# togatoga/kanpyo

Measured on AMD Instinct MI355X. Metric: sentences/sec, higher is better.
Workload: dtype i32; 1 GPU; BASELINE configs[1] (cfg 2): 100k synthetic ~40-char sentences, batch 4096, IPADIC-shaped 392k-record dictionary; batch=4096, batches_in_flight=8, streams=3, long_streams=0, GPU_MAX_HW_QUEUES=4, residency=inputs resident in HBM, dense tokens left in HBM

## Files before the change

### kanpyo_amd/csrc/kgpu_chain.cpp

```cpp
#include "kgpu_chain.h"

#include <algorithm>
#include <cstdlib>

namespace kgpu {

LaunchPlan make_launch_plan(int cus, const Occupancy &occ) {
    LaunchPlan t{};
    t.general_workgroups = cus * 2;
    const char *e = getenv("KGPU_POOL");
    t.pool_limit_auto = e == nullptr;
    for (const char *q = e ? e : "40:4:32"; *q && t.n_pools < 2;) {
        int kib = atoi(q), w = 8, mp = 64;
        const char *c = q;
        while (*c && *c != ',' && *c != ':') ++c;
        if (*c == ':' && atoi(c + 1) > 0) {
            w = atoi(c + 1);
            ++c;
            while (*c && *c != ',' && *c != ':') ++c;
            if (*c == ':' && atoi(c + 1) > 0) mp = atoi(c + 1);
        }
        w = std::min(w, 16);
        mp = std::min(mp, 64);
        const int per_cu = kib >= 8 && kib <= 160 ? occ.pool((uint32_t)kib * 1024, (uint32_t)w) : 0;
        if (per_cu > 0) {
            t.pool_bytes[t.n_pools] = (uint32_t)kib * 1024; t.pool_waves[t.n_pools] = (uint32_t)w;
            t.pool_max_pages[t.n_pools] = (uint32_t)mp;
            t.pool_workgroups[t.n_pools] = cus * per_cu;
            ++t.n_pools;
        }
        while (*q && *q != ',') ++q;
        if (*q == ',') ++q;
    }
    t.alt_pool_bytes = 20 * 1024; t.alt_pool_waves = 2;
    const int alt_per_cu = (t.pool_limit_auto && t.n_pools) ? occ.pool(t.alt_pool_bytes, t.alt_pool_waves) : 0;
    t.alt_pool_workgroups = alt_per_cu > 0 ? cus * alt_per_cu : 0;
    const char *w = getenv("KGPU_WINDOW");
    int kib = w ? atoi(w) : 10;
    if (kib < 8 || kib > 160) kib = 0;
    t.window_lds_bytes = (uint32_t)kib * 1024;
    const int per_cu = kib ? occ.window(t.window_lds_bytes) : 0;
    t.window_workgroups = cus * per_cu;
    if (per_cu <= 0) t.window_lds_bytes = 0;
    t.window_team_workgroups = t.window_lds_bytes ? cus * std::max(0, occ.window_team(t.window_lds_bytes)) : 0;
    const char *tm = getenv("KGPU_WINDOW_TEAM");
    t.window_team_mode = tm ? atoi(tm) : -1;
    const char *wf = getenv("KGPU_WINDOW_FIRST");
    t.window_first_bytes = (uint32_t)std::max(0, wf ? atoi(wf) : 1024);
    return t;
}

int Chain::pools() const {
    int k = 0;
    while (k < n && steps[k].kernel == Kernel::Pool) ++k;
    return k;
}
const Step *Chain::find(Kernel k) const {
    for (int i = 0; i < n; ++i) if (steps[i].kernel == k) return &steps[i];
    return nullptr;
}

bool starts_with_window(const LaunchPlan &plan, const Batch &b) {
    const uint64_t lim = plan.window_first_bytes;
    return lim && b.n && plan.n_pools && plan.window_lds_bytes && !b.dump && b.stop_after == 0 && !b.no_window && b.bytes >= lim * b.n;
}

static Step window_step(const LaunchPlan &plan, uint64_t n, int in, int out, int grid_est) {
    uint64_t wg = plan.window_workgroups;
    if (in < 0 && n < wg) wg = n;
    if (in >= 0 && grid_est > 0 && (uint64_t)grid_est < wg) wg = (uint64_t)grid_est;
    const uint64_t expected = in >= 0 ? (grid_est > 64 ? ((uint64_t)grid_est - 64) * 4 / 5 : 0) : n;
    return Step{Kernel::Window, in, out, (int)(wg ? wg : 1), plan.window_lds_bytes, 1, 0, expected > wg};
}
static Step general_step(const LaunchPlan &plan, uint64_t n, int in) {
    uint64_t wg = plan.general_workgroups;
    if (in < 0 && n < wg) wg = n;
    return Step{Kernel::General, in, -1, (int)(wg ? wg : 1), 0, 0, 0, false};
}

Chain build_chain(const LaunchPlan &plan, const Batch &b, Steering &st, ContextSteering &cs) {
    Chain ch;
    if (!b.n) return ch;
    const int pools = starts_with_window(plan, b) ? 0 : st.big_pool_batches.load(std::memory_order_relaxed) > 0 ? plan.n_pools : std::min(plan.n_pools, 1);
    const bool window = plan.window_lds_bytes && !b.no_window && !b.dump && b.stop_after == 0 &&
                        (pools == 0 || st.window_batches.load(std::memory_order_relaxed) > 0);
    const bool general = (pools == 0 && !window) || b.stop_after != 0 || b.dump || b.no_window || st.tail_batches.load(std::memory_order_relaxed) > 0;
    bool team = false;
    if (pools == 0 && window && plan.window_team_workgroups > 0 && plan.window_team_mode != 0) {
// ... 79 lines not shown
```

### kanpyo_amd/csrc/kgpu_chain.h

```cpp
#pragma once
#include <atomic>
#include <cstdint>

#include "kgpu_internal.h"

namespace kgpu {

struct LaunchPlan {
    int n_pools;
    uint32_t pool_bytes[2];
    uint32_t pool_waves[2];
    uint32_t pool_max_pages[2];
    bool pool_limit_auto;
    uint32_t alt_pool_bytes, alt_pool_waves;
    int alt_pool_workgroups;
    int pool_workgroups[2];
    int general_workgroups;
    uint32_t window_lds_bytes;
    int window_workgroups;
    int window_team_workgroups;
    int window_team_mode;
    uint32_t window_first_bytes;
};

struct Occupancy {
    int (*pool)(uint32_t pool_bytes, uint32_t waves);
    int (*window)(uint32_t lds_bytes);
    int (*window_team)(uint32_t lds_bytes);
};
LaunchPlan make_launch_plan(int compute_units, const Occupancy &occ);

enum class Kernel : uint8_t { Pool, WindowTeam, Window, General };
struct Step {
    Kernel kernel;
    int in;
    int out;
    int grid;
    uint32_t lds_bytes;
    uint32_t waves;
    uint32_t max_pages;
    bool claim;
};

struct Chain {
    Step steps[4];
    int n = 0;
    bool event_behind_first = false;
    bool small_scan = false;
    bool aux_one_launch = false;
    int pools() const;
    const Step *find(Kernel k) const;
    int last_list() const { return n ? steps[n - 1].out : -1; }
};

constexpr uint64_t AUX_ONE_LAUNCH_MAX = 4096;

struct Batch {
    uint64_t n, bytes;
    uint32_t est_q8;
    uint32_t stop_after;
    bool dump;
    bool no_window;
    bool share_known;
};

struct Steering {
    std::atomic<uint32_t> est_q8{64 * 256};
    std::atomic<int> big_pool_batches{0};
    std::atomic<int> window_batches{64};
    std::atomic<int> tail_batches{0};
    std::atomic<int> long_sentences_in_flight{0};
    std::atomic<int> long_peak{0};
};
struct ContextSteering {
    uint32_t win_share_q8 = 0;
    bool long_share = false;
    int counted_long = 0;
};

bool starts_with_window(const LaunchPlan &plan, const Batch &b);
Chain build_chain(const LaunchPlan &plan, const Batch &b, Steering &st, ContextSteering &cs);
Chain tail_chain(const LaunchPlan &plan, const Chain &ran);
void chain_feedback(const LaunchPlan &plan, const Chain &ran, const Chain *tail, const Control &h, uint64_t n, uint32_t est_q8, Steering &st,
                    ContextSteering &cs);

}
```

### kanpyo_amd/csrc/kgpu_ctx.cpp

```cpp
#include <algorithm>
#include <cstdlib>
#include <cstring>
#include <mutex>
#include <vector>

#include "kgpu_runtime.h"


extern "C" int kgpu_ctx_create(kgpu_dict *d, void *hip_stream, kgpu_ctx **out) {
    if (!d || !out) { set_error("kgpu_ctx_create: null argument"); return KGPU_ERR_INVALID_ARG; }
    *out = nullptr;
    HIPCHECK(hipSetDevice(d->device));
    kgpu_ctx *c = new kgpu_ctx();
    c->dict = d;
    d->refs.fetch_add(1, std::memory_order_relaxed);
    if (hip_stream) { c->stream = (hipStream_t)hip_stream; c->own_stream = true; }
    else {
        std::lock_guard<std::mutex> g(d->pool_mu);
        const unsigned n_streams = planned_streams();
        if (d->streams.size() < n_streams) {
            hipStream_t st = nullptr;
            hipError_t e = hipStreamCreateWithFlags(&st, hipStreamNonBlocking);
            if (e != hipSuccess) { set_error("hipStreamCreate: %s", hipGetErrorString(e)); kgpu_ctx_destroy(c); return KGPU_ERR_HIP; }
            d->streams.push_back(st);
            c->stream = st;
        } else {
            c->stream = d->streams[d->next_stream++ % d->streams.size()];
        }
        c->short_stream = c->stream;
    }
    if (hipMalloc((void **)&c->d_ctl, sizeof(Control)) != hipSuccess ||
        hipHostMalloc((void **)&c->h_ctl, sizeof(Control), hipHostMallocMapped) != hipSuccess ||
        hipHostGetDevicePointer((void **)&c->h_ctl_dev, c->h_ctl, 0) != hipSuccess) {
        set_error("kgpu_ctx_create: control block allocation failed");
        kgpu_ctx_destroy(c);
        return KGPU_ERR_HIP;
    }
    if (hipEventCreateWithFlags(&c->done_ev, hipEventDisableTiming) != hipSuccess || hipEventCreateWithFlags(&c->switch_ev, hipEventDisableTiming) != hipSuccess) {
        set_error("kgpu_ctx_create: hipEventCreate failed");
        kgpu_ctx_destroy(c);
        return KGPU_ERR_HIP;
    }
    hipDeviceProp_t p;
    const int cus = hipGetDeviceProperties(&p, d->device) == hipSuccess ? p.multiProcessorCount : 256;
    c->plan = make_launch_plan(cus, Occupancy{pool_workgroups_per_cu, window_workgroups_per_cu, window_team_workgroups_per_cu});
    c->aux_mode = test_hooks().aux_launch;
    *out = c;
    return KGPU_OK;
}

static void ctx_retire(kgpu_ctx *c) {
    c->pending = false;
    if (c->steer.counted_long) { c->dict->steer.long_sentences_in_flight.fetch_sub(c->steer.counted_long, std::memory_order_relaxed); c->steer.counted_long = 0; }
}

extern "C" void kgpu_ctx_destroy(kgpu_ctx *c) {
    if (!c) return;
    (void)hipSetDevice(c->dict->device);
    if (c->pending && c->done_ev) (void)hipEventSynchronize(c->done_ev);
    ctx_retire(c);
    if (c->done_ev) (void)hipEventDestroy(c->done_ev);
    c->lines_report.release(); c->split_report.release();
    c->lines_len.release(); c->lines_text.release(); c->lines_off.release(); c->lines_status.release();
    c->split_agg.release(); c->split_raw.release(); c->split_text.release(); c->split_off.release();
    c->gv_desc.release(); c->gv_len.release(); c->gv_text.release(); c->norm_text.release();
    if (c->switch_ev) (void)hipEventDestroy(c->switch_ev);
    for (auto e : c->ev_pool) (void)hipEventDestroy(e);
    c->arena.release(); c->ovf.release(); c->stat_slots.release(); c->stage.release(); c->tok_count.release();
    c->in_utf8.release(); c->in_off.release(); c->out_tok.release(); c->out_off.release(); c->out_status.release();
    c->pin_in.release(); c->pin_out.release(); c->in_block.release();
    if (c->d_ctl) (void)hipFree(c->d_ctl);
    if (c->h_ctl) (void)hipHostFree(c->h_ctl);
    if (c->sm_host) (void)hipHostFree(c->sm_host);
    kgpu_dict *d = c->dict;
    delete c;
    dict_release(d);
}

static int next_event(kgpu_ctx *c, hipEvent_t *ev) {
    if (c->ev_used == c->ev_pool.size()) {
        hipEvent_t e;
        HIPCHECK(hipEventCreate(&e));
        c->ev_pool.push_back(e);
    }
    *ev = c->ev_pool[c->ev_used++];
    return KGPU_OK;
}

static int ctx_pick_stream(kgpu_ctx *c, const Batch &b) {
    if (c->own_stream) { c->h2d_queued = false; return KGPU_OK; }
    hipStream_t want = c->short_stream;
    if ((starts_with_window(c->plan, b) || c->steer.long_share) && planned_long_streams()) {
        if (!c->long_stream) {
            kgpu_dict *d = c->dict;
            std::lock_guard<std::mutex> g(d->pool_mu);
            if (d->long_streams.size() < planned_long_streams()) {
                hipStream_t st = nullptr;
                if (hipStreamCreateWithFlags(&st, hipStreamNonBlocking) == hipSuccess) d->long_streams.push_back(st);
                else (void)hipGetLastError();
            }
            if (!d->long_streams.empty()) c->long_stream = d->long_streams[d->next_long++ % d->long_streams.size()];
        }
        if (c->long_stream) want = c->long_stream;
    }
    if (want != c->stream) {
        if (c->h2d_queued) {
            HIPCHECK(hipEventRecord(c->switch_ev, c->stream));
            HIPCHECK(hipStreamWaitEvent(want, c->switch_ev, 0));
        }
        c->stream = want;
    }
    c->h2d_queued = false;
    return KGPU_OK;
}

static int run_chain(kgpu_ctx *c, const BatchArgs &a, const hipEvent_t *ev, const char *what) {
    const Chain &ch = c->chain;
    if (ev && !ch.event_behind_first) HIPCHECK(hipEventRecord(ev[0], c->stream));
    for (int k = 0; k < ch.n; ++k) {
        hipError_t e = (hipError_t)launch_step(c->dict->view, a, ch.steps[k], c->stop_after, c->stream);
        if (e == hipSuccess && ev && k == 0 && ch.event_behind_first) e = hipEventRecord(ev[0], c->stream);
        if (e != hipSuccess) { set_error("%s launch: %s", what, hipGetErrorString(e)); return KGPU_ERR_HIP; }
    }
    if (ev) HIPCHECK(hipEventRecord(ev[1], c->stream));
    c->h_ctl->pack_overflow = 0;
    hipError_t e = (hipError_t)launch_scan_compact(a, c->h_ctl_dev, c->stream, ch.small_scan, ch.aux_one_launch, c->aux_mode, &c->aux_form);
    if (e != hipSuccess) { set_error("scan/compact launch: %s", hipGetErrorString(e)); return KGPU_ERR_HIP; }
    if (ev) HIPCHECK(hipEventRecord(ev[2], c->stream));
    HIPCHECK(hipEventRecord(c->done_ev, c->stream));
    c->ctl_dirty = false;
    c->pending = true;
    return KGPU_OK;
}

static int enqueue(kgpu_ctx *c, const BatchArgs &a, const Batch &b) {
    if (c->ctl_dirty) HIPCHECK(hipMemsetAsync(c->d_ctl, 0, sizeof(Control), c->stream));
    c->ctl_dirty = true;
    hipEvent_t ev[4] = {};
    int rc;
    const bool timed = c->profiling && (c->launch_seq++ % c->event_every) == 0;
    if (timed) {
        for (hipEvent_t &e : ev) if ((rc = next_event(c, &e))) return rc;
        HIPCHECK(hipEventRecord(ev[0], c->stream));
    }
    c->chain = build_chain(c->plan, b, c->dict->steer, c->steer);
    c->last = a;
    return run_chain(c, a, timed ? ev + 1 : nullptr, "k_tokenize");
}

int kgpu::tokenize_device_impl(kgpu_ctx *c, const uint8_t *d_utf8, const uint64_t *d_offsets, uint64_t n, uint64_t total_bytes,
                                kgpu_token *d_tokens, kgpu_token8 *d_tokens8, uint32_t *d_first, uint8_t *status8, uint64_t *toff8, uint64_t token_capacity,
                                uint64_t *d_tok_offsets, uint8_t *d_status, const char *who) {
    if (!c || !d_offsets || !d_tok_offsets || (n && !d_status) || (total_bytes && !d_utf8) ||
        (token_capacity && !d_tokens && !d_tokens8) || (d_tokens8 && n && !d_first)) {
        set_error("%s: null argument", who);
        return KGPU_ERR_INVALID_ARG;
    }
    if (n >= (1ull << 32) - 1) { set_error("%s: more than 2^32-2 sentences in one batch; split it", who); return KGPU_ERR_INVALID_ARG; }
    if (total_bytes >= (1ull << 32)) { set_error("%s: batch larger than 4 GiB; split it", who); return KGPU_ERR_INVALID_ARG; }
    HIPCHECK(hipSetDevice(c->dict->device));
    int rc;
    if (c->pending && (rc = kgpu_ctx_sync(c, nullptr)) != KGPU_OK && rc != KGPU_ERR_CAPACITY) return rc;
    const Batch b{n, total_bytes, c->dict->steer.est_q8.load(std::memory_order_relaxed), c->stop_after, false, false, c->rt.batches > 0};
    if ((rc = ctx_pick_stream(c, b))) return rc;
    if ((rc = c->arena.ensure(ARENA_INITIAL)) || (rc = c->stage.ensure((size_t)token_bound(total_bytes, n) * sizeof(kgpu_token) + 64)) ||
        (rc = c->tok_count.ensure((size_t)(n + 1) * 4)) ||
        (rc = c->ovf.ensure((size_t)(n + 1) * 4 * 4)))
        return rc;
    BatchArgs a{};
    a.utf8 = d_utf8; a.offsets = d_offsets; a.n = n; a.ctl = c->d_ctl;
    a.arena = (uint8_t *)c->arena.p; a.arena_bytes = c->arena.bytes;
    a.stage = (kgpu_token *)c->stage.p;
    a.tok_count = (uint32_t *)c->tok_count.p;
    a.status = d_status; a.out = d_tokens; a.out_cap = token_capacity; a.tok_offsets = d_tok_offsets;
    a.out8 = d_tokens8; a.first8 = d_first; a.status8 = status8; a.toff8 = toff8;
    a.count_work = c->count_work ? (c->count_no_t ? 3u : 1u) : 0u;
#ifdef KGPU_STEP_TIMING
    const bool want_stats = true;
#else
    const bool want_stats = c->count_work;
#endif
    if (want_stats) {
        if (!c->stat_slots.p) {
            if ((rc = c->stat_slots.ensure((size_t)STAT_SLOTS * STAT_WORDS * 8))) return rc;
            HIPCHECK(hipMemsetAsync(c->stat_slots.p, 0, (size_t)STAT_SLOTS * STAT_WORDS * 8, c->stream));
        }
        a.stat_slots = (unsigned long long *)c->stat_slots.p;
    }
    a.est_q8 = b.est_q8;
    for (int k = 0; k < 4; ++k) a.ovf[k] = (uint32_t *)c->ovf.p + (size_t)k * (n + 1);
    c->batch = b;
    return enqueue(c, a, b);
}

static int enqueue_tail(kgpu_ctx *c, int li) {
    HIPCHECK(hipMemcpyAsync(&c->d_ctl->ovf_count[li], &c->tail_saved.ovf_count[li], sizeof(unsigned), hipMemcpyHostToDevice, c->stream));
    c->ctl_dirty = true;
    return run_chain(c, c->last, nullptr, "tail");
}

extern "C" int kgpu_tokenize_device(kgpu_ctx *c, const uint8_t *d_utf8, const uint64_t *d_offsets, uint64_t n,
                                    uint64_t total_bytes, kgpu_token *d_tokens, uint64_t token_capacity,
                                    uint64_t *d_tok_offsets, uint8_t *d_status) {
    return tokenize_device_impl(c, d_utf8, d_offsets, n, total_bytes, d_tokens, nullptr, nullptr, nullptr, nullptr, token_capacity, d_tok_offsets, d_status,
                                "kgpu_tokenize_device");
}

extern "C" int kgpu_tokenize_device_compact(kgpu_ctx *c, const uint8_t *d_utf8, const uint64_t *d_offsets, uint64_t n,
                                            uint64_t total_bytes, kgpu_token8 *d_tokens8, uint64_t token_capacity,
                                            uint32_t *d_first, uint64_t *d_tok_offsets, uint8_t *d_status) {
    if (token_capacity && !d_tokens8) { set_error("kgpu_tokenize_device_compact: null argument"); return KGPU_ERR_INVALID_ARG; }
    return tokenize_device_impl(c, d_utf8, d_offsets, n, total_bytes, nullptr, d_tokens8, d_first, nullptr, nullptr, token_capacity, d_tok_offsets, d_status,
                                "kgpu_tokenize_device_compact");
}

extern "C" void kgpu_expand_tokens(const kgpu_token8 *in, const uint64_t *tok_offsets, const uint32_t *first, uint64_t n, kgpu_token *out) {
    const bool stream = n && expand_stream_wanted(tok_offsets[n] - tok_offsets[0]);
    expand_tokens(in, tok_offsets, first, n, out, stream);
    if (stream) expand_fence();
}

extern "C" int kgpu_ctx_sync(kgpu_ctx *c, uint64_t *n_tokens) {
    if (!c) { set_error("kgpu_ctx_sync: null ctx"); return KGPU_ERR_INVALID_ARG; }
    HIPCHECK(hipSetDevice(c->dict->device));
    for (;;) {
        if (!c->pending) { if (n_tokens) *n_tokens = 0; return KGPU_OK; }
        HIPCHECK(hipEventSynchronize(c->done_ev));
        if (c->h_ctl->window_fail && !c->h_ctl->arena_overflow) {
            c->rt.window_reruns++;
            if (c->last.stat_slots) HIPCHECK(hipMemsetAsync(c->last.stat_slots, 0, (size_t)STAT_SLOTS * STAT_WORDS * 8, c->stream));
            c->tail_pass = false;
            Batch b = c->batch;
            b.no_window = true;
            int rc = enqueue(c, c->last, b);
            if (rc) { ctx_retire(c); return rc; }
            continue;
        }
        const int li = c->chain.last_list();
        if (li >= 0 && !c->h_ctl->arena_overflow && c->h_ctl->ovf_count[li] > 0) {
            c->rt.tail_reruns++;
            c->tail_saved = *c->h_ctl;
            c->tail_pass = true;
            c->first_pass = c->chain;
            c->chain = tail_chain(c->plan, c->first_pass);
            int rc = enqueue_tail(c, li);
            if (rc) { ctx_retire(c); c->tail_pass = false; return rc; }
            continue;
        }
        if (c->h_ctl->arena_overflow) {
            size_t want = c->arena.bytes * 2;
            if (want > ARENA_MAX) { set_error("scratch arena exceeded %zu bytes", ARENA_MAX); ctx_retire(c); return KGPU_ERR_INTERNAL; }
            int rc = c->arena.ensure(want);
            if (rc) { ctx_retire(c); return rc; }
            BatchArgs a = c->last;
            a.arena = (uint8_t *)c->arena.p; a.arena_bytes = c->arena.bytes;
            c->rt.arena_regrows++;
            c->tail_pass = false;
            if (a.stat_slots) HIPCHECK(hipMemsetAsync(a.stat_slots, 0, (size_t)STAT_SLOTS * STAT_WORDS * 8, c->stream));
            if ((rc = enqueue(c, a, c->batch))) { ctx_retire(c); return rc; }
            continue;
        }
        break;
    }
    ctx_retire(c);
    const Chain &first = c->tail_pass ? c->first_pass : c->chain;
    const Chain *tail = c->tail_pass ? &c->chain : nullptr;
    if (c->tail_pass) {
        c->tail_pass = false;
        Control &h = *c->h_ctl;
        const Control &sv = c->tail_saved;
        for (int k = 0; k < 4; ++k) { if (k <= first.last_list()) h.ovf_count[k] = sv.ovf_count[k]; h.late_count[k] += sv.late_count[k]; }
        for (int k = 0; k < 7; ++k) h.work[k] += sv.work[k];
        for (int k = 0; k < 10; ++k) h.phase[k] += sv.phase[k];
        h.pack_overflow |= sv.pack_overflow;
    }
    c->rt.batches++; c->rt.sentences += c->last.n;
    for (int k = 0; k < 4; ++k) { c->rt.deferred[k] += c->h_ctl->ovf_count[k]; c->rt.redone[k] += c->h_ctl->late_count[k]; }
    if (first.find(Kernel::Window) || (tail && tail->find(Kernel::Window))) c->rt.long_launches++;
    chain_feedback(c->plan, first, tail, *c->h_ctl, c->last.n, c->last.est_q8, c->dict->steer, c->steer);
    if (c->profiling) {
        for (size_t i = 0; i + 4 <= c->ev_used; i += 4) {
            float t0f = 0, t01 = 0, t12 = 0;
            if (hipEventElapsedTime(&t0f, c->ev_pool[i], c->ev_pool[i + 1]) == hipSuccess &&
                hipEventElapsedTime(&t01, c->ev_pool[i], c->ev_pool[i + 2]) == hipSuccess &&
                hipEventElapsedTime(&t12, c->ev_pool[i + 2], c->ev_pool[i + 3]) == hipSuccess) {
                c->prof.launches++; c->rt.first_ms += t0f; c->prof.tokenize_ms += t01; c->prof.aux_ms += t12;
            }
        }
        c->ev_used = 0;
    }
    if (c->last.count_work) {
        const unsigned long long *w = c->h_ctl->work;
        c->work.sentences += w[0]; c->work.B += w[1]; c->work.C += w[2]; c->work.T += w[3];
        c->work.N += w[4]; c->work.E += w[5]; c->work.K += w[6];
        for (int k = 0; k < 10; ++k) c->phase[k] += c->h_ctl->phase[k];
    }
    if (c->last.stat_slots) {
        const size_t words = (size_t)STAT_SLOTS * STAT_WORDS;
        c->stat_host.resize(words);
        HIPCHECK(hipMemcpyAsync(c->stat_host.data(), c->last.stat_slots, words * 8, hipMemcpyDeviceToHost, c->stream));
        HIPCHECK(hipMemsetAsync(c->last.stat_slots, 0, words * 8, c->stream));
        HIPCHECK(hipStreamSynchronize(c->stream));
        unsigned long long sum[STAT_WORDS] = {0};
        for (size_t i = 0; i < words; ++i) sum[i % STAT_WORDS] += c->stat_host[i];
        c->work.sentences += sum[0]; c->work.B += sum[1]; c->work.C += sum[2]; c->work.T += sum[3];
        c->work.N += sum[4]; c->work.E += sum[5]; c->work.K += sum[6];
        for (int k = 0; k < 10; ++k) c->phase[k] += sum[16 + k];
    }
    uint64_t need = c->h_ctl->n_tokens;
    if (c->last.out8 && c->h_ctl->pack_overflow) {
        if (n_tokens) *n_tokens = 0;
        set_error("a token does not fit the 8-byte record (more than 4095 chars or 262143 bytes): use the 24-byte form for this batch");
        return KGPU_ERR_CAPACITY;
    }
    if (n_tokens) *n_tokens = need;
    if (c->h_ctl->n_tokens > c->last.out_cap) {
        set_error("token buffer too small: need %llu, capacity %llu", (unsigned long long)need, (unsigned long long)c->last.out_cap);
        return KGPU_ERR_CAPACITY;
    }
    return KGPU_OK;
}

extern "C" int kgpu_debug_aux_form(kgpu_ctx *c) { return c ? c->aux_form : -1; }

extern "C" int kgpu_ctx_set_profiling(kgpu_ctx *c, int mode) {
    if (!c) { set_error("kgpu_ctx_set_profiling: null ctx"); return KGPU_ERR_INVALID_ARG; }
    c->profiling = (mode & KGPU_PROFILE_EVENTS) != 0;
    c->event_every = (mode & KGPU_PROFILE_SAMPLED) ? 4u : 1u;
    c->launch_seq = 0;
    c->count_work = (mode & KGPU_PROFILE_WORK) != 0;
    c->count_no_t = (mode & KGPU_PROFILE_NO_T) != 0;
    return KGPU_OK;
}

extern "C" int kgpu_ctx_set_ablation(kgpu_ctx *c, int stop_after_stage) {
    if (!c || stop_after_stage < 0 || stop_after_stage > 7) { set_error("kgpu_ctx_set_ablation: bad argument"); return KGPU_ERR_INVALID_ARG; }
    c->stop_after = (uint32_t)stop_after_stage;
    return KGPU_OK;
}

extern "C" int kgpu_ctx_get_phase_cycles(kgpu_ctx *c, uint64_t out[10], int reset) {
    if (!c || !out) { set_error("kgpu_ctx_get_phase_cycles: null argument"); return KGPU_ERR_INVALID_ARG; }
    for (int k = 0; k < 10; ++k) { out[k] = c->phase[k]; if (reset) c->phase[k] = 0; }
    return KGPU_OK;
}

extern "C" int kgpu_ctx_get_work(kgpu_ctx *c, kgpu_work *out, int reset) {
    if (!c || !out) { set_error("kgpu_ctx_get_work: null argument"); return KGPU_ERR_INVALID_ARG; }
    *out = c->work;
    if (reset) c->work = kgpu_work{};
    return KGPU_OK;
}

extern "C" int kgpu_ctx_get_profile(kgpu_ctx *c, kgpu_profile *out, int reset) {
    if (!c || !out) { set_error("kgpu_ctx_get_profile: null argument"); return KGPU_ERR_INVALID_ARG; }
    *out = c->prof;
    if (reset) c->prof = kgpu_profile{};
    return KGPU_OK;
}

extern "C" int kgpu_ctx_get_plan(kgpu_ctx *c, kgpu_plan_info *out, size_t out_size) {
    if (!c || !out || out_size < 4) { set_error("kgpu_ctx_get_plan: bad argument"); return KGPU_ERR_INVALID_ARG; }
    HIPCHECK(hipSetDevice(c->dict->device));
    kgpu_plan_info p{};
    hipDeviceProp_t prop;
    p.compute_units = hipGetDeviceProperties(&prop, c->dict->device) == hipSuccess ? (uint32_t)prop.multiProcessorCount : 0u;
    if (c->plan.n_pools) {
        p.pool_lds_bytes = c->plan.pool_bytes[0]; p.pool_wavefronts = c->plan.pool_waves[0]; p.pool_max_pages = c->plan.pool_max_pages[0];
        p.pool_workgroups_per_cu = (uint32_t)pool_workgroups_per_cu(c->plan.pool_bytes[0], c->plan.pool_waves[0]);
    }
    p.window_lds_bytes = c->plan.window_lds_bytes; p.window_workgroups = (uint32_t)c->plan.window_workgroups;
    p.window_workgroups_per_cu = c->plan.window_lds_bytes ? (uint32_t)window_workgroups_per_cu(c->plan.window_lds_bytes) : 0u;
    p.streams = planned_streams();
    p.long_streams = c->own_stream ? 0u : planned_long_streams();
    p.window_first_bytes = (c->plan.n_pools && c->plan.window_lds_bytes) ? c->plan.window_first_bytes : 0u;
    std::memcpy(out, &p, std::min(out_size, sizeof p));
    return KGPU_OK;
}

extern "C" int kgpu_ctx_get_routing(kgpu_ctx *c, kgpu_routing *out, size_t out_size, int reset) {
    if (!c || !out || out_size < 8) { set_error("kgpu_ctx_get_routing: bad argument"); return KGPU_ERR_INVALID_ARG; }
    std::memcpy(out, &c->rt, std::min(out_size, sizeof(kgpu_routing)));
    if (reset) c->rt = kgpu_routing{};
    return KGPU_OK;
}

int HostReport::arm() {
    if (pending) { pending = false; HIPCHECK(hipEventSynchronize(ev)); }
    if (int rc = ctl.ensure(16, true)) return rc;
    if (!ev) HIPCHECK(hipEventCreateWithFlags(&ev, hipEventDisableTiming));
    unsigned long long *h = (unsigned long long *)ctl.h;
    h[0] = 0; h[1] = 0;
    return KGPU_OK;
}
int HostReport::record(hipStream_t stream, uint64_t cap_) {
    HIPCHECK(hipEventRecord(ev, stream));
    pending = true;
    cap = cap_;
    return KGPU_OK;
}
int HostReport::wait(uint64_t words[2]) {
    pending = false;
    HIPCHECK(hipEventSynchronize(ev));
    const unsigned long long *h = (const unsigned long long *)ctl.h;
    words[0] = h[0]; words[1] = h[1];
    return KGPU_OK;
// ... 1 lines not shown
void HostReport::release() {
    if (pending && ev) (void)hipEventSynchronize(ev);
    if (ev) (void)hipEventDestroy(ev);
    ev = nullptr; pending = false;
    ctl.release();
}

int kgpu::require_features(kgpu_dict *d, const char *who) {
    std::lock_guard<std::mutex> g(d->feat_mu);
    if (!d->feat) { set_error("%s: the dictionary has no feature tables: call kgpu_dict_set_features first", who); return KGPU_ERR_INVALID_ARG; }
    return KGPU_OK;
}
int kgpu::begin_records_call(kgpu_ctx *c, const char *who) {
    if (c->pending) { set_error("%s: the context's tokenize batch is not synced (kgpu_ctx_sync) yet", who); return KGPU_ERR_INVALID_ARG; }
    HIPCHECK(hipSetDevice(c->dict->device));
    int rc;
    if (c->lines_report.pending && (rc = kgpu_ctx_sync_lines(c, nullptr)) != KGPU_OK && rc != KGPU_ERR_CAPACITY) return rc;
    return KGPU_OK;
}
int kgpu::records_batch(kgpu_ctx *c, const DeviceRecords &r, size_t scratch_bytes, uint64_t *d_unit_offsets, RecordsBatch &b) {
    int rc;
    if ((rc = c->lines_report.arm()) || (rc = c->lines_len.ensure(scratch_bytes))) return rc;
    const kgpu_dict_info &di = c->dict->info;
    b = RecordsBatch{r.d_utf8, r.d_offsets, r.n, r.d_tokens, r.d_tok_offsets, (uint32_t)di.n_morphs, (uint32_t)(di.n_morphs + di.n_unk_morphs),
                     (uint64_t *)c->lines_len.p, d_unit_offsets, r.status_in, r.status_out, c->lines_report.dev()};
    return KGPU_OK;
}
int kgpu::records_launched(kgpu_ctx *c, int launch_error, const char *who, const char *what, uint64_t capacity) {
    if (launch_error != (int)hipSuccess) { set_error("%s: %s launch: %s", who, what, hipGetErrorString((hipError_t)launch_error)); return KGPU_ERR_HIP; }
    return c->lines_report.record(c->stream, capacity);
}
int kgpu::enqueue_lines(kgpu_ctx *c, const DeviceRecords &r, uint8_t *d_text, uint64_t text_capacity, uint64_t *d_text_offsets, const char *who) {
    kgpu_dict *d = c->dict;
    LinesArgs a{};
    int rc;
    if ((rc = require_features(d, who)) || (rc = records_batch(c, r, (size_t)r.n * 8 + 8, d_text_offsets, a.b))) return rc;
    a.feat = d->feat; a.feat_off = d->feat_off;
    a.text = d_text; a.text_cap = text_capacity;
    return records_launched(c, launch_format_lines(a, c->stream), who, "render", text_capacity);
}

extern "C" int kgpu_format_lines_device(kgpu_ctx *c, const uint8_t *d_utf8, const uint64_t *d_offsets, uint64_t n,
                                        const kgpu_token *d_tokens, const uint64_t *d_tok_offsets,
                                        uint8_t *d_text, uint64_t text_capacity, uint64_t *d_text_offsets) {
    const char *who = "kgpu_format_lines_device";
    if (!c || !d_offsets || !d_tok_offsets || !d_text_offsets || (n && (!d_utf8 || !d_tokens)) || (text_capacity && !d_text)) {
        set_error("%s: null argument", who);
        return KGPU_ERR_INVALID_ARG;
    }
    if (int rc = begin_records_call(c, who)) return rc;
    return enqueue_lines(c, DeviceRecords{d_utf8, d_offsets, n, d_tokens, d_tok_offsets, nullptr, nullptr}, d_text, text_capacity, d_text_offsets, who);
}

extern "C" int kgpu_ctx_sync_lines(kgpu_ctx *c, uint64_t *n_bytes) {
    if (!c) { set_error("kgpu_ctx_sync_lines: null ctx"); return KGPU_ERR_INVALID_ARG; }
    if (!c->lines_report.pending) { if (n_bytes) *n_bytes = 0; return KGPU_OK; }
    HIPCHECK(hipSetDevice(c->dict->device));
    uint64_t h[2];
    if (int rc = c->lines_report.wait(h)) return rc;
    const uint64_t need = h[0];
    if (n_bytes) *n_bytes = need;
    if (h[1]) {
        set_error("kgpu_ctx_sync_lines: a token record names a class, morph id or surface outside the dictionary or its sentence");
        return KGPU_ERR_INVALID_ARG;
    }
    if (need > c->lines_report.cap) {
        set_error("text buffer too small: need %llu, capacity %llu", (unsigned long long)need, (unsigned long long)c->lines_report.cap);
        return KGPU_ERR_CAPACITY;
    }
    return KGPU_OK;
}

int kgpu::pool_get(kgpu_dict *d, kgpu_ctx **out) {
    kgpu_ctx *c = nullptr;
    {
        std::lock_guard<std::mutex> g(d->pool_mu);
        if (!d->pool.empty()) { c = d->pool.back(); d->pool.pop_back(); }
    }
    if (!c) { int rc = kgpu_ctx_create(d, nullptr, &c); if (rc) return rc; }
    *out = c;
    return KGPU_OK;
}
void kgpu::pool_put(kgpu_dict *d, kgpu_ctx *c) {
    std::lock_guard<std::mutex> g(d->pool_mu);
    d->pool.push_back(c);
}

int kgpu::ctx_h2d(kgpu_ctx *c, void *dst, const void *src, size_t bytes, const char *what) {
    const hipError_t e = hipMemcpyAsync(dst, src, bytes, hipMemcpyHostToDevice, c->stream);
    if (e != hipSuccess) { set_error("%s: %s", what, hipGetErrorString(e)); return KGPU_ERR_HIP; }
    c->h2d_queued = true;
    return KGPU_OK;
}

extern "C" int kgpu_lattice_dump(kgpu_dict *d, const uint8_t *utf8, uint64_t len, kgpu_lattice *out) {
    if (!d || !out || (len && !utf8)) { set_error("kgpu_lattice_dump: null argument"); return KGPU_ERR_INVALID_ARG; }
    if (len >= (1ull << 31)) { set_error("kgpu_lattice_dump: sentence too long"); return KGPU_ERR_INVALID_ARG; }
    *out = kgpu_lattice{};
    HIPCHECK(hipSetDevice(d->device));
    PooledCtx lease(d);
    kgpu_ctx *c = lease.c;
    int rc = lease.rc;
    if (rc) return rc;
    const uint64_t offs[2] = {0, len};
    Control hc{};
    if ((c->pending && (rc = kgpu_ctx_sync(c, nullptr)) != KGPU_OK && rc != KGPU_ERR_CAPACITY) ||
        (rc = c->arena.ensure(ARENA_INITIAL)) || (rc = c->stage.ensure((size_t)(len + 2) * sizeof(kgpu_token) + 64)) ||
        (rc = c->tok_count.ensure(8)) || (rc = c->in_utf8.ensure((size_t)len + 16)) || (rc = c->in_off.ensure(16)) ||
        (rc = c->out_status.ensure(16))) return rc;
    auto fail = [&](hipError_t e, const char *what) { set_error("kgpu_lattice_dump: %s: %s", what, hipGetErrorString(e)); c->ctl_dirty = true; return KGPU_ERR_HIP; };
    hipError_t e;
    if (len && (e = hipMemcpyAsync(c->in_utf8.p, utf8, (size_t)len, hipMemcpyHostToDevice, c->stream)) != hipSuccess) return fail(e, "H2D");
    if ((e = hipMemcpyAsync(c->in_off.p, offs, 16, hipMemcpyHostToDevice, c->stream)) != hipSuccess) return fail(e, "H2D");
    for (;;) {
        BatchArgs a{};
        a.utf8 = (const uint8_t *)c->in_utf8.p; a.offsets = (const uint64_t *)c->in_off.p; a.n = 1; a.ctl = c->d_ctl;
        a.arena = (uint8_t *)c->arena.p; a.arena_bytes = c->arena.bytes;
        a.stage = (kgpu_token *)c->stage.p; a.tok_count = (uint32_t *)c->tok_count.p; a.status = (uint8_t *)c->out_status.p;
        a.dump_lattice = 1;
        c->ctl_dirty = true;
        if ((e = hipMemsetAsync(c->d_ctl, 0, sizeof(Control), c->stream)) != hipSuccess) return fail(e, "memset");
        if ((e = (hipError_t)launch_general_only(d->view, a, c->stream)) != hipSuccess) return fail(e, "launch");
        if ((e = hipMemcpyAsync(&hc, c->d_ctl, sizeof(Control), hipMemcpyDeviceToHost, c->stream)) != hipSuccess) return fail(e, "D2H");
        if ((e = hipStreamSynchronize(c->stream)) != hipSuccess) return fail(e, "sync");
        if (!hc.arena_overflow) break;
        size_t want = c->arena.bytes * 2;
        if (want > ARENA_MAX) { set_error("scratch arena exceeded %zu bytes", ARENA_MAX); return KGPU_ERR_INTERNAL; }
        if ((rc = c->arena.ensure(want))) return rc;
    }
    if (!hc.dump[5]) { set_error("kgpu_lattice_dump: the sentence is not valid UTF-8"); return KGPU_ERR_INVALID_ARG; }
    const uint64_t B = hc.dump[2], C = hc.dump[3], N = hc.dump[4], na = B + 4;
    std::vector<uint32_t> cbyte(C + 1), boff(C + 2), pre(N);
    std::vector<uint32_t> nodeA(4 * N), bucket(4 * N), nodeB(2 * N);
    const uint8_t *sa = (const uint8_t *)c->arena.p + hc.dump[0], *sn = (const uint8_t *)c->arena.p + hc.dump[1];
    if ((e = hipMemcpy(cbyte.data(), sa, (C + 1) * 4, hipMemcpyDeviceToHost)) != hipSuccess ||
        (e = hipMemcpy(boff.data(), sa + 3 * na * 4, (C + 2) * 4, hipMemcpyDeviceToHost)) != hipSuccess ||
        (e = hipMemcpy(nodeA.data(), sn, N * 16, hipMemcpyDeviceToHost)) != hipSuccess ||
        (e = hipMemcpy(bucket.data(), sn + N * 16, N * 16, hipMemcpyDeviceToHost)) != hipSuccess ||
        (e = hipMemcpy(nodeB.data(), sn + N * 32, N * 8, hipMemcpyDeviceToHost)) != hipSuccess ||
        (e = hipMemcpy(pre.data(), sn + N * 40, N * 4, hipMemcpyDeviceToHost)) != hipSuccess) return fail(e, "slab read-back");
    lease.put();
    out->n_nodes = N; out->n_positions = C + 2;
    out->nodes = (kgpu_lattice_node *)calloc((size_t)N, sizeof(kgpu_lattice_node));
    out->edge_offsets = (uint32_t *)calloc((size_t)C + 3, 4);
    out->edge_nodes = (uint32_t *)calloc((size_t)N, 4);
    if (!out->nodes || !out->edge_offsets || !out->edge_nodes) { kgpu_lattice_free(out); set_error("kgpu_lattice_dump: out of memory"); return KGPU_ERR_INTERNAL; }
    auto orig = [](const std::vector<uint32_t> &inv, uint32_t r) { return (int16_t)(inv.empty() || r >= inv.size() ? r : inv[r]); };
    for (uint64_t t = 0; t < N; ++t) {
        kgpu_lattice_node &nd = out->nodes[t];
        if (t == 0) { nd.pre = -1; continue; }
        const uint32_t *A = &nodeA[4 * t];
        const int32_t sid = (int32_t)A[3];
        const uint32_t st = nodeB[2 * t], en = nodeB[2 * t + 1];
        nd.id = sid < 0 ? -sid : sid;
        nd.cls = sid > 0 ? KGPU_CLASS_KNOWN : sid < 0 ? KGPU_CLASS_UNKNOWN : KGPU_CLASS_DUMMY;
        nd.char_pos = st; nd.end_char = en; nd.byte_pos = cbyte[st]; nd.byte_len = cbyte[en] - cbyte[st];
        if (sid != 0) { nd.left_id = orig(d->left_of_rank, A[0] & 0xFFFFu); nd.right_id = orig(d->right_of_rank, A[0] >> 16); nd.cost = (int16_t)(int32_t)A[1]; }
        nd.dp = A[2] == 0xFFFFFFFFu ? (int32_t)hc.dump[6] : (int32_t)bucket[4 * A[2]];
        nd.pre = pre[t] == 0xFFFFFFFFu ? -1 : (int32_t)pre[t];
    }
    for (uint64_t e2 = 0; e2 <= C + 1; ++e2) out->edge_offsets[e2] = e2 <= C + 1 && e2 < boff.size() ? boff[e2] : 0;
    out->edge_offsets[C + 1] = (uint32_t)(N - 1); out->edge_offsets[C + 2] = (uint32_t)N;
    for (uint64_t sl = 0; sl + 1 < N; ++sl) out->edge_nodes[sl] = bucket[4 * sl + 2];
    out->edge_nodes[N - 1] = (uint32_t)(N - 1);
    for (uint64_t e2 = 0; e2 <= C; ++e2) std::sort(out->edge_nodes + out->edge_offsets[e2], out->edge_nodes + out->edge_offsets[e2 + 1]);
    return KGPU_OK;
}

extern "C" void kgpu_lattice_free(kgpu_lattice *l) {
    if (!l) return;
    free(l->nodes); free(l->edge_offsets); free(l->edge_nodes);
// ... 3 lines not shown
```

### kanpyo_amd/csrc/kgpu_runtime.h

```cpp
#pragma once
#include <hip/hip_runtime_api.h>

#include <atomic>
#include <cstdlib>
#include <condition_variable>
#include <deque>
#include <functional>
#include <mutex>
#include <shared_mutex>
#include <thread>
#include <vector>

#include "kgpu_chain.h"

#define HIPCHECK(expr)                                                                  \
    do {                                                                                \
        hipError_t e_ = (expr);                                                         \
        if (e_ != hipSuccess) {                                                         \
            set_error("%s failed: %s (%s:%d)", #expr, hipGetErrorString(e_), __FILE__, __LINE__); \
            return KGPU_ERR_HIP;                                                        \
        }                                                                               \
    } while (0)

namespace kgpu {

struct DevBuf {
    void *p = nullptr; size_t bytes = 0;
    int ensure(size_t need) {
        if (need <= bytes) return KGPU_OK;
        if (p) { (void)hipFree(p); p = nullptr; bytes = 0; }
        size_t want = need + need / 4 + 256;
        HIPCHECK(hipMalloc(&p, want));
        bytes = want;
        return KGPU_OK;
    }
    void release() { if (p) (void)hipFree(p); p = nullptr; bytes = 0; }
};

struct PinBuf {
    void *h = nullptr, *d = nullptr; size_t bytes = 0;
    int ensure(size_t need, bool mapped) {
        if (need <= bytes) return KGPU_OK;
        release();
        size_t want = need + need / 4 + 4096;
        if (hipHostMalloc(&h, want, mapped ? hipHostMallocMapped : hipHostMallocDefault) != hipSuccess) { h = nullptr; set_error("pinned allocation of %zu bytes failed", want); return KGPU_ERR_HIP; }
        d = h;
        if (mapped && hipHostGetDevicePointer(&d, h, 0) != hipSuccess) { (void)hipHostFree(h); h = d = nullptr; set_error("hipHostGetDevicePointer failed"); return KGPU_ERR_HIP; }
        bytes = want;
        return KGPU_OK;
    }
    void release() { if (h) (void)hipHostFree(h); h = d = nullptr; bytes = 0; }
};

struct HostReport {
    PinBuf ctl;
    hipEvent_t ev = nullptr;
    bool pending = false;
    uint64_t cap = 0;
    int arm();
    unsigned long long *dev() const { return (unsigned long long *)ctl.d; }
    int record(hipStream_t stream, uint64_t cap);
    int wait(uint64_t words[2]);
    void release();
};

}

using namespace kgpu;

struct Combiner;

struct kgpu_dict {
    int device = 0;
    Combiner *combiner = nullptr;
    int combiner_callers() const;
    DictView view{};
    kgpu_dict_info info{};
    std::vector<void *> allocs;
    std::mutex pool_mu;
    std::vector<kgpu_ctx *> pool;
    Steering steer;
    std::vector<hipStream_t> streams;
    unsigned next_stream = 0;
    std::vector<hipStream_t> long_streams;
    unsigned next_long = 0;
    std::vector<uint32_t> left_of_rank, right_of_rank;
    std::mutex feat_mu;
    const uint8_t *feat = nullptr;
    const uint32_t *feat_off = nullptr;
    std::vector<uint8_t> label_host;
    std::vector<uint32_t> label_off_host;
    const uint8_t *label = nullptr;
    const uint32_t *label_off = nullptr;
    std::vector<uint8_t> feat_blob_known, feat_blob_unk;
    std::mutex keys_mu;
    bool keys_built = false;
    std::vector<DaNode> da_host;
    std::vector<std::pair<int64_t, uint64_t>> dup_host;
    std::vector<uint8_t> key_bytes;
    std::vector<uint64_t> key_off;
    bool norm_ready = false;
    NormTables norm{};
    std::atomic<int> refs{1};
    std::atomic<bool> closed{false};
};

struct kgpu_words {
    kgpu_dict *dict = nullptr;
    int32_t field = -1;
    uint32_t filter = 0, sep = ' ';
    void *d_rows = nullptr, *d_names = nullptr;
    std::vector<WordRow> h_rows;
    std::vector<uint8_t> h_names;
    std::atomic<int> refs{1};
};

struct kgpu_counts {
    kgpu_words *words = nullptr;
    uint64_t table_slots = 0, key_bytes = 0;
    void *d_dense = nullptr, *d_slots = nullptr, *d_arena = nullptr, *d_stats = nullptr;
    std::shared_mutex mu;
    std::atomic<uint64_t> sentences{0};
    std::atomic<uint64_t> version{1};
    uint64_t cached_version = 0;
    std::vector<uint8_t> cached_words;
    std::vector<uint64_t> cached_off, cached_counts;
};

struct kgpu_vocab {
    kgpu_words *words = nullptr;
    uint32_t flags = 0;
    int32_t unk_id = 0, bos_id = 0, eos_id = 0;
    uint64_t n_words = 0, table_slots = 0, key_bytes = 0, rows_resolved = 0;
    void *d_row_id = nullptr, *d_slots = nullptr, *d_arena = nullptr;
    bool wordpiece = false, cont_shared = false;
    uint32_t max_word_chars = 0, initial_max = 0, cont_max = 0;
    void *d_cont_slots = nullptr, *d_cont_arena = nullptr, *d_wp_rows = nullptr, *d_piece_ids = nullptr;
    kgpu_wordpiece_info wp{};
};

struct kgpu_ctx {
    kgpu_dict *dict = nullptr;
    hipStream_t stream = nullptr;
    hipStream_t short_stream = nullptr, long_stream = nullptr;
    bool own_stream = false;
    ContextSteering steer;
    bool h2d_queued = false;
    hipEvent_t switch_ev = nullptr;
    hipEvent_t done_ev = nullptr;
    Control *d_ctl = nullptr;
    Control *h_ctl = nullptr;
    Control *h_ctl_dev = nullptr;
    bool ctl_dirty = true;
    uint32_t launch_seq = 0;
    Batch batch{};
    Chain chain;
    bool tail_pass = false;
    Chain first_pass;
    Control tail_saved{};
    uint32_t event_every = 1;
    DevBuf arena, stage, tok_count;
    DevBuf in_utf8, in_off, out_tok, out_off, out_status;
    PinBuf pin_in, pin_out;
    DevBuf in_block;
    uint8_t *sm_host = nullptr, *sm_dev = nullptr;
    uint32_t sm_seq = 0;
    DevBuf lines_len;
    HostReport lines_report;
    PinBuf lines_text, lines_off, lines_status;
    DevBuf gv_desc, gv_len, gv_text;
    DevBuf split_agg, split_raw, split_text, split_off;
    HostReport split_report;
    DevBuf norm_text;
    BatchArgs last{};
    bool pending = false;
    LaunchPlan plan{};
    int aux_form = 0;
    int aux_mode = -1;
    DevBuf ovf;
    DevBuf stat_slots;
    std::vector<unsigned long long> stat_host;
    bool profiling = false;
    bool count_work = false;
    bool count_no_t = false;
    uint32_t stop_after = 0;
    kgpu_work work{};
    uint64_t phase[10] = {0};
    std::vector<hipEvent_t> ev_pool;
    size_t ev_used = 0;
    kgpu_profile prof{};
    kgpu_routing rt{};
};


#if defined(__x86_64__)
#include <immintrin.h>
#endif

namespace kgpu {

inline void expand_tokens(const kgpu_token8 *in, const uint64_t *tok_offsets, const uint32_t *first, uint64_t n, kgpu_token *out, bool stream) {
    const uint64_t base = tok_offsets[0];
#if defined(__x86_64__)
    if (stream && ((uintptr_t)out & 7u) == 0) {
        for (uint64_t s = 0; s < n; ++s) {
            uint32_t pos = first[2 * s], st = first[2 * s + 1];
            for (uint64_t k = tok_offsets[s] - base, e = tok_offsets[s + 1] - base; k < e; ++k) {
                const uint32_t p = in[k].packed, chars = KGPU_T8_CHARS(p), bytes = KGPU_T8_BYTES(p);
                long long *o = (long long *)(out + k);
                _mm_stream_si64(o, (long long)((uint64_t)(uint32_t)in[k].id | ((uint64_t)KGPU_T8_CLS(p) << 32)));
                _mm_stream_si64(o + 1, (long long)((uint64_t)pos | ((uint64_t)st << 32)));
                _mm_stream_si64(o + 2, (long long)((uint64_t)(st + chars) | ((uint64_t)bytes << 32)));
                pos += bytes; st += chars;
            }
        }
        return;
    }
#endif
    for (uint64_t s = 0; s < n; ++s) {
        uint32_t pos = first[2 * s], st = first[2 * s + 1];
        for (uint64_t k = tok_offsets[s] - base, e = tok_offsets[s + 1] - base; k < e; ++k) {
            const uint32_t p = in[k].packed, chars = KGPU_T8_CHARS(p), bytes = KGPU_T8_BYTES(p);
            out[k] = kgpu_token{in[k].id, KGPU_T8_CLS(p), pos, st, st + chars, bytes};
            pos += bytes; st += chars;
        }
    }
}
inline void expand_fence() {
#if defined(__x86_64__)
    _mm_sfence();
#endif
}
constexpr uint64_t EXPAND_STREAM_MIN_TOKENS = 32768;
inline bool expand_stream_wanted(uint64_t tokens) {
    static const int mode = [] { const char *e = getenv("KGPU_EXPAND_STREAM"); return e ? atoi(e) : -1; }();
    return mode >= 0 ? mode != 0 : tokens >= EXPAND_STREAM_MIN_TOKENS;
}

struct WorkerPool {
    std::mutex mu; std::condition_variable cv; std::deque<std::function<void()>> q; std::vector<std::thread> th;
    std::mutex done_mu; std::condition_variable done_cv;
    unsigned start();
    void submit(std::function<void()> f);
    void wait_zero(std::atomic<int> &counter);
    void task_done(std::atomic<int> &counter);
};
WorkerPool &workers();
struct TestHooks { bool no_small_calls = false, plain_leaves = false, byte_trie = false; uint64_t chunk_bytes = 4ull << 20, chunk_sents = 16384, depth = 12, multi_chunk_sents = 0, graphviz_chunk_sents = 0, graphviz_arena_initial = 0, graphviz_arena_max = 0; int aux_launch = -1; };
TestHooks test_hooks();
bool env_flag_now(const char *name);

unsigned planned_streams();
unsigned planned_long_streams();
void dict_release(kgpu_dict *d);

constexpr size_t ARENA_INITIAL = 1ull << 28;
constexpr size_t ARENA_MAX = 1ull << 37;
int pool_get(kgpu_dict *d, kgpu_ctx **c);
void pool_put(kgpu_dict *d, kgpu_ctx *c);
struct PooledCtx {
    kgpu_dict *d = nullptr; kgpu_ctx *c = nullptr; int rc = KGPU_OK;
    PooledCtx() = default;
    explicit PooledCtx(kgpu_dict *d_) { get(d_); }
    PooledCtx(const PooledCtx &) = delete; PooledCtx &operator=(const PooledCtx &) = delete;
    ~PooledCtx() { put(); }
    int get(kgpu_dict *d_) { d = d_; return rc = pool_get(d, &c); }
    void put() { if (c) { c->h2d_queued = false; pool_put(d, c); c = nullptr; } }
};
int ctx_h2d(kgpu_ctx *c, void *dst, const void *src, size_t bytes, const char *what);
int tokenize_device_impl(kgpu_ctx *c, const uint8_t *d_utf8, const uint64_t *d_offsets, uint64_t n, uint64_t total_bytes,
                         kgpu_token *d_tokens, kgpu_token8 *d_tokens8, uint32_t *d_first, uint8_t *status8, uint64_t *toff8, uint64_t token_capacity,
                         uint64_t *d_tok_offsets, uint8_t *d_status, const char *who);
struct DeviceRecords {
    const uint8_t *d_utf8; const uint64_t *d_offsets; uint64_t n; const kgpu_token *d_tokens; const uint64_t *d_tok_offsets;
    const uint8_t *status_in; uint8_t *status_out;
};
int begin_records_call(kgpu_ctx *c, const char *who);
int records_batch(kgpu_ctx *c, const DeviceRecords &r, size_t scratch_bytes, uint64_t *d_unit_offsets, RecordsBatch &b);
int records_launched(kgpu_ctx *c, int launch_error, const char *who, const char *what, uint64_t capacity);
WordTable word_table(const kgpu_words *w);
int enqueue_lines(kgpu_ctx *c, const DeviceRecords &r, uint8_t *d_text, uint64_t text_capacity, uint64_t *d_text_offsets, const char *who);
int enqueue_words(kgpu_ctx *c, const kgpu_words *w, const DeviceRecords &r, uint8_t *d_text, uint64_t text_capacity, uint64_t *d_text_offsets, const char *who);
int build_word_table(const uint8_t *known, size_t known_len, const uint8_t *unk, size_t unk_len, uint64_t n_morphs, uint64_t n_unk,
                     const kgpu_words_spec &spec, std::vector<WordRow> &rows, std::vector<uint8_t> &names);

void words_release(kgpu_words *w);
int enqueue_encode(kgpu_ctx *c, const kgpu_vocab *v, const DeviceRecords &r, int32_t *d_ids, uint64_t id_capacity, uint64_t width, int32_t pad_id, uint64_t *d_id_offsets, const char *who);
void dict_key_table(kgpu_dict *d);
int enqueue_count(kgpu_ctx *c, kgpu_counts *k, const DeviceRecords &r, const char *who);

int enqueue_normalize(kgpu_ctx *c, int form, const uint8_t *d_utf8, const uint64_t *d_offsets, uint64_t n, uint8_t *d_text, uint64_t text_capacity,
                      uint64_t *d_text_offsets, uint8_t *d_status, const char *who);

int require_features(kgpu_dict *d, const char *who);
int ensure_label_pool(kgpu_dict *d);

void parallel_copy(void *dst, const void *src, size_t bytes);
bool is_pinned_host(const void *p);
int batch_depth();
bool batch_is_pinned(const uint8_t *utf8, const uint64_t *offsets, uint64_t n);
int check_host_batch(const char *who, const uint64_t *offsets, uint64_t n, const uint8_t *utf8);
inline uint64_t token_bound(uint64_t total, uint64_t n) { return total + n + 1; }
struct MergeSrc { const kgpu_token8 *rec; const uint32_t *first; const uint64_t *toff; const uint8_t *st; };
struct ChunkInput {
    uint64_t n = 0, total = 0;
    size_t in_off = 0;
    int prepare(kgpu_ctx *c, uint64_t n, uint64_t total, bool staged);
    const uint64_t *d_offsets(const kgpu_ctx *c) const { return (const uint64_t *)c->in_block.p; }
    const uint8_t *d_text(const kgpu_ctx *c, uint64_t base) const { return (const uint8_t *)c->in_block.p + in_off - base; }
};
int upload_input(kgpu_ctx *c, const ChunkInput &in, const uint8_t *utf8, const uint64_t *off, bool pinned_in);
int split_block(kgpu_ctx *sc, const uint8_t *text, uint64_t len, const char *who, std::vector<uint64_t> &off, uint64_t &lines);
struct ChunkBlock {
    ChunkInput in;
    uint64_t cap = 0;
    size_t off_first = 0, off_toff = 0, off_status = 0;
    int prepare(kgpu_ctx *c, uint64_t n, uint64_t total, bool staged);
    int launch(kgpu_ctx *c, uint64_t base, const char *who) const;
    MergeSrc results(const kgpu_ctx *c) const;
};
struct LinesSink {
    uint8_t *text; uint64_t text_capacity; uint64_t *text_offsets; uint8_t *status;
    bool status_after_overflow;
    uint64_t text_done = 0;
    bool overflow = false;
    uint64_t unit = 1;
};
struct Renderer {
    enum Kind { LINES, WORDS, IDS } kind = LINES;
    const kgpu_words *words = nullptr;
    const kgpu_vocab *vocab = nullptr;
    Renderer() = default;
    explicit Renderer(const kgpu_words *w) : kind(WORDS), words(w) {}
    explicit Renderer(const kgpu_vocab *v) : kind(IDS), vocab(v) {}
    uint64_t unit() const { return kind == IDS ? 4 : 1; }
    const char *noun() const { return kind == IDS ? "id" : "text"; }
    size_t first_bytes(uint64_t total, uint64_t n) const;
    int enqueue(kgpu_ctx *c, const DeviceRecords &r, void *d_out, size_t out_bytes, uint64_t *d_offsets, const char *who) const;
};
struct RecordsChunk {
    uint64_t n = 0, total = 0;
    const uint8_t *d_utf8 = nullptr;
    const uint64_t *d_offsets = nullptr;
    int prepare(kgpu_ctx *c, uint64_t n, uint64_t total);
    int launch(kgpu_ctx *c, const char *who) const;
    DeviceRecords records(const kgpu_ctx *c) const;
};
struct LinesChunk : RecordsChunk {
    Renderer renderer;
    int prepare(kgpu_ctx *c, uint64_t n, uint64_t total);
// ... 87 lines not shown
```

Before: 138.3 million sentences/s.

## Assign each batch to the least-loaded HIP stream instead of fixed round-robin

```diff
diff --git a/kanpyo_amd/csrc/kgpu_chain.cpp b/kanpyo_amd/csrc/kgpu_chain.cpp
--- a/kanpyo_amd/csrc/kgpu_chain.cpp
+++ b/kanpyo_amd/csrc/kgpu_chain.cpp
@@ -4,6 +4,20 @@
 #include <cstdlib>
 
 namespace kgpu {
+
+unsigned pick_stream(const std::atomic<uint64_t> *load, unsigned n, std::atomic<unsigned> &cursor) {
+    if (n <= 1) return 0;
+    const unsigned from = cursor.load(std::memory_order_relaxed) % n;
+    unsigned best = from;
+    uint64_t least = load[from].load(std::memory_order_relaxed);
+    for (unsigned k = 1; k < n && least; ++k) {
+        const unsigned i = (from + k) % n;
+        const uint64_t l = load[i].load(std::memory_order_relaxed);
+        if (l + l / STREAM_TIE_SHARE < least) { least = l; best = i; }
+    }
+    cursor.store((best + 1) % n, std::memory_order_relaxed);
+    return best;
+}
 
 LaunchPlan make_launch_plan(int cus, const Occupancy &occ) {
     LaunchPlan t{};
diff --git a/kanpyo_amd/csrc/kgpu_chain.h b/kanpyo_amd/csrc/kgpu_chain.h
--- a/kanpyo_amd/csrc/kgpu_chain.h
+++ b/kanpyo_amd/csrc/kgpu_chain.h
@@ -84,4 +84,9 @@
 void chain_feedback(const LaunchPlan &plan, const Chain &ran, const Chain *tail, const Control &h, uint64_t n, uint32_t est_q8, Steering &st,
                     ContextSteering &cs);
 
+constexpr uint64_t STREAM_BATCH_BASE = 256;
+inline uint64_t stream_batch_weight(uint64_t total_bytes) { return total_bytes + STREAM_BATCH_BASE; }
+constexpr uint64_t STREAM_TIE_SHARE = 8;
+unsigned pick_stream(const std::atomic<uint64_t> *load, unsigned n, std::atomic<unsigned> &cursor);
+
 }
diff --git a/kanpyo_amd/csrc/kgpu_ctx.cpp b/kanpyo_amd/csrc/kgpu_ctx.cpp
--- a/kanpyo_amd/csrc/kgpu_ctx.cpp
+++ b/kanpyo_amd/csrc/kgpu_ctx.cpp
@@ -18,16 +18,20 @@
     else {
         std::lock_guard<std::mutex> g(d->pool_mu);
         const unsigned n_streams = planned_streams();
-        if (d->streams.size() < n_streams) {
+        if (!d->stream_load) {
+            d->stream_load.reset(new std::atomic<uint64_t>[n_streams]);
+            d->stream_batches.reset(new std::atomic<uint64_t>[n_streams]);
+            for (unsigned k = 0; k < n_streams; ++k) { d->stream_load[k].store(0, std::memory_order_relaxed); d->stream_batches[k].store(0, std::memory_order_relaxed); }
+            d->streams.reserve(n_streams);
+        }
+        while (d->streams.size() < n_streams) {
             hipStream_t st = nullptr;
             hipError_t e = hipStreamCreateWithFlags(&st, hipStreamNonBlocking);
             if (e != hipSuccess) { set_error("hipStreamCreate: %s", hipGetErrorString(e)); kgpu_ctx_destroy(c); return KGPU_ERR_HIP; }
             d->streams.push_back(st);
-            c->stream = st;
-        } else {
-            c->stream = d->streams[d->next_stream++ % d->streams.size()];
-        }
-        c->short_stream = c->stream;
+        }
+        c->short_idx = pick_stream(d->stream_load.get(), n_streams, d->stream_cursor);
+        c->stream = c->short_stream = d->streams[c->short_idx];
     }
     if (hipMalloc((void **)&c->d_ctl, sizeof(Control)) != hipSuccess ||
         hipHostMalloc((void **)&c->h_ctl, sizeof(Control), hipHostMallocMapped) != hipSuccess ||
@@ -51,6 +55,7 @@
 
 static void ctx_retire(kgpu_ctx *c) {
     c->pending = false;
+    if (c->load_weight) { c->dict->stream_load[c->load_idx].fetch_sub(c->load_weight, std::memory_order_relaxed); c->load_weight = 0; }
     if (c->steer.counted_long) { c->dict->steer.long_sentences_in_flight.fetch_sub(c->steer.counted_long, std::memory_order_relaxed); c->steer.counted_long = 0; }
 }
 
@@ -87,7 +92,29 @@
     return KGPU_OK;
 }
 
+static void ctx_begin_batch(kgpu_ctx *c) {
+    if (c->batch_begun) return;
+    c->batch_begun = true;
+    if (c->own_stream || c->pending || c->lines_report.pending || c->split_report.pending) return;
+    kgpu_dict *d = c->dict;
+    const bool on_short = c->stream == c->short_stream;
+    c->short_idx = pick_stream(d->stream_load.get(), (unsigned)d->streams.size(), d->stream_cursor);
+    c->short_stream = d->streams[c->short_idx];
+    if (on_short) c->stream = c->short_stream;
+}
+
+static void ctx_count_load(kgpu_ctx *c, uint64_t total_bytes) {
+    if (c->own_stream || c->stream != c->short_stream || c->load_weight) return;
+    kgpu_dict *d = c->dict;
+    c->load_idx = c->short_idx;
+    c->load_weight = stream_batch_weight(total_bytes);
+    d->stream_load[c->load_idx].fetch_add(c->load_weight, std::memory_order_relaxed);
+    d->stream_batches[c->load_idx].fetch_add(1, std::memory_order_relaxed);
+}
+
 static int ctx_pick_stream(kgpu_ctx *c, const Batch &b) {
+    ctx_begin_batch(c);
+    c->batch_begun = false;
     if (c->own_stream) { c->h2d_queued = false; return KGPU_OK; }
     hipStream_t want = c->short_stream;
     if ((starts_with_window(c->plan, b) || c->steer.long_share) && planned_long_streams()) {
@@ -148,9 +175,24 @@
     return run_chain(c, a, timed ? ev + 1 : nullptr, "k_tokenize");
 }
 
+static int tokenize_batch(kgpu_ctx *c, const uint8_t *d_utf8, const uint64_t *d_offsets, uint64_t n, uint64_t total_bytes,
+                          kgpu_token *d_tokens, kgpu_token8 *d_tokens8, uint32_t *d_first, uint8_t *status8, uint64_t *toff8, uint64_t token_capacity,
+                          uint64_t *d_tok_offsets, uint8_t *d_status, const char *who);
+
 int kgpu::tokenize_device_impl(kgpu_ctx *c, const uint8_t *d_utf8, const uint64_t *d_offsets, uint64_t n, uint64_t total_bytes,
                                 kgpu_token *d_tokens, kgpu_token8 *d_tokens8, uint32_t *d_first, uint8_t *status8, uint64_t *toff8, uint64_t token_capacity,
                                 uint64_t *d_tok_offsets, uint8_t *d_status, const char *who) {
+    const int rc = tokenize_batch(c, d_utf8, d_offsets, n, total_bytes, d_tokens, d_tokens8, d_first, status8, toff8, token_capacity, d_tok_offsets, d_status, who);
+    if (rc && c) {
+        if (c->h2d_queued && !c->pending) (void)hipStreamSynchronize(c->stream);
+        c->batch_begun = c->h2d_queued = false;
+    }
+    return rc;
+}
+
+static int tokenize_batch(kgpu_ctx *c, const uint8_t *d_utf8, const uint64_t *d_offsets, uint64_t n, uint64_t total_bytes,
+                          kgpu_token *d_tokens, kgpu_token8 *d_tokens8, uint32_t *d_first, uint8_t *status8, uint64_t *toff8, uint64_t token_capacity,
+                          uint64_t *d_tok_offsets, uint8_t *d_status, const char *who) {
     if (!c || !d_offsets || !d_tok_offsets || (n && !d_status) || (total_bytes && !d_utf8) ||
         (token_capacity && !d_tokens && !d_tokens8) || (d_tokens8 && n && !d_first)) {
         set_error("%s: null argument", who);
@@ -190,7 +232,9 @@
     a.est_q8 = b.est_q8;
     for (int k = 0; k < 4; ++k) a.ovf[k] = (uint32_t *)c->ovf.p + (size_t)k * (n + 1);
     c->batch = b;
-    return enqueue(c, a, b);
+    if ((rc = enqueue(c, a, b))) return rc;
+    ctx_count_load(c, total_bytes);
+    return KGPU_OK;
 }
 
 static int enqueue_tail(kgpu_ctx *c, int li) {
@@ -322,6 +366,17 @@
 }
 
 extern "C" int kgpu_debug_aux_form(kgpu_ctx *c) { return c ? c->aux_form : -1; }
+extern "C" int kgpu_debug_stream_batches(kgpu_dict *d, uint64_t *out, int cap, int reset) {
+    if (!d) return -1;
+    std::lock_guard<std::mutex> g(d->pool_mu);
+    const int n = (int)d->streams.size();
+    if (!d->stream_batches || n < (int)planned_streams()) return 0;
+    for (int k = 0; k < n; ++k) {
+        const uint64_t v = reset ? d->stream_batches[k].exchange(0, std::memory_order_relaxed) : d->stream_batches[k].load(std::memory_order_relaxed);
+        if (out && k < cap) out[k] = v;
+    }
+    return n;
+}
 
 extern "C" int kgpu_ctx_set_profiling(kgpu_ctx *c, int mode) {
     if (!c) { set_error("kgpu_ctx_set_profiling: null ctx"); return KGPU_ERR_INVALID_ARG; }
@@ -489,11 +544,13 @@
     return KGPU_OK;
 }
 void kgpu::pool_put(kgpu_dict *d, kgpu_ctx *c) {
+    c->batch_begun = c->h2d_queued = false;
     std::lock_guard<std::mutex> g(d->pool_mu);
     d->pool.push_back(c);
 }
 
 int kgpu::ctx_h2d(kgpu_ctx *c, void *dst, const void *src, size_t bytes, const char *what) {
+    ctx_begin_batch(c);
     const hipError_t e = hipMemcpyAsync(dst, src, bytes, hipMemcpyHostToDevice, c->stream);
     if (e != hipSuccess) { set_error("%s: %s", what, hipGetErrorString(e)); return KGPU_ERR_HIP; }
     c->h2d_queued = true;
diff --git a/kanpyo_amd/csrc/kgpu_runtime.h b/kanpyo_amd/csrc/kgpu_runtime.h
--- a/kanpyo_amd/csrc/kgpu_runtime.h
+++ b/kanpyo_amd/csrc/kgpu_runtime.h
@@ -6,6 +6,7 @@
 #include <condition_variable>
 #include <deque>
 #include <functional>
+#include <memory>
 #include <mutex>
 #include <shared_mutex>
 #include <thread>
@@ -81,7 +82,8 @@
     std::vector<kgpu_ctx *> pool;
     Steering steer;
     std::vector<hipStream_t> streams;
-    unsigned next_stream = 0;
+    std::unique_ptr<std::atomic<uint64_t>[]> stream_load, stream_batches;
+    std::atomic<unsigned> stream_cursor{0};
     std::vector<hipStream_t> long_streams;
     unsigned next_long = 0;
     std::vector<uint32_t> left_of_rank, right_of_rank;
@@ -143,8 +145,12 @@
     kgpu_dict *dict = nullptr;
     hipStream_t stream = nullptr;
     hipStream_t short_stream = nullptr, long_stream = nullptr;
+    unsigned short_idx = 0;
+    uint64_t load_weight = 0;
+    unsigned load_idx = 0;
     bool own_stream = false;
     ContextSteering steer;
+    bool batch_begun = false;
     bool h2d_queued = false;
     hipEvent_t switch_ev = nullptr;
     hipEvent_t done_ev = nullptr;
@@ -265,7 +271,7 @@
     PooledCtx(const PooledCtx &) = delete; PooledCtx &operator=(const PooledCtx &) = delete;
     ~PooledCtx() { put(); }
     int get(kgpu_dict *d_) { d = d_; return rc = pool_get(d, &c); }
-    void put() { if (c) { c->h2d_queued = false; pool_put(d, c); c = nullptr; } }
+    void put() { if (c) { pool_put(d, c); c = nullptr; } }
 };
 int ctx_h2d(kgpu_ctx *c, void *dst, const void *src, size_t bytes, const char *what);
 int tokenize_device_impl(kgpu_ctx *c, const uint8_t *d_utf8, const uint64_t *d_offsets, uint64_t n, uint64_t total_bytes,
```

New measurement: 149.9 million sentences/s, median of 6. 1.08x the previous value.
